# EasyVision-Ton/VMG

Measured on AMD Instinct MI355X. Metric: LR-frames/s (train: forward+loss+backward+AdamW), VMG-REDS-few_levels 4x SR, higher is better.
Workload: dtype bf16; 1 GPU; VMG-REDS-few_levels train step, per-GPU batch 4x7x3x64x64 -> 4x SR (BASELINE configs[1]); global_batch=4, frames_per_clip=7, parallelism=dp1, launch=eager, recompute_chains=False, fp8_chains=False

## Files before the change

### include/vmg_hip.h

```cpp
#ifndef VMG_HIP_H
#define VMG_HIP_H

#include <stdint.h>

#ifdef __cplusplus
extern "C" {
#endif

#define VMG_F32 0
#define VMG_BF16 1

#define VMG_ACT_NONE 0
#define VMG_ACT_RELU 1
#define VMG_ACT_LRELU 2
#define VMG_ACT_GELU 3

#define VMG_CONV_GENERAL 0
#define VMG_CONV_KSPLIT 2
#define VMG_CONV_WS 3
#define VMG_CONV_LINEAR_WRES 4
#define VMG_CONV_WSTAT 6

const char* vmg_last_error(void);
int vmg_version(void);

typedef struct vmg_ctx vmg_ctx;
vmg_ctx* vmg_create(int device);
int vmg_destroy(vmg_ctx* ctx);
int vmg_ctx_device(const vmg_ctx* ctx);
int vmg_max_lds_bytes(void);

int64_t vmg_conv_pack_bytes(int dtype, int ks, int on, int nsrc, const int* src_ch, int cout_tiles);
int vmg_conv_pack(int dtype, const float* w, int O, int I, int ks, int o0, int on, int nsrc, const int* src_off,
                  const int* src_ch, int transpose_flip, int cout_tiles, void* packed, void* stream);

int64_t vmg_convws_pack_bytes(int on, int nsrc, const int* src_ch, int cout_tiles);
int vmg_convws_pack(const float* w, int O, int I, int o0, int on, int nsrc, const int* src_off, const int* src_ch, int transpose_flip,
                    int cout_tiles, void* packed, void* stream);

typedef struct vmg_conv_desc {
  int dtype, ks, cout_tiles;
  int N, H, W, Cout;
  int nsrc;
  const void* src[4];
  int64_t src_ps[4];
  int src_ch[4];
  const void* packed;
  const float* bias;
  void* out;
  int64_t out_ps;
  void* out_pre;
  const void* res;
  int64_t res_ps;
  const void* aux;
// ... 269 lines not shown
```

### vmg_amd/csrc/conv_igemm.hip

```cpp
#include <stdlib.h>

#include <type_traits>

#include "common.h"

namespace {

constexpr int MAX_ISRC = 32;
constexpr int CBMAX = 160;

__host__ __device__ constexpr int kstg(int ks) { return ks > 1 ? ks : 2; }
__host__ __device__ constexpr int stage_bytes(int ks, int ntb, int cb) { return kstg(ks) * 4 * ntb * 16 * cb; }
__host__ __device__ constexpr int stage_stride(int ks, int ntb, int cb) { return (stage_bytes(ks, ntb, cb) + 4095) / 4096 * 4096; }
__host__ __device__ inline int stages_of(int ks, int ch) {
  const int nb = (ch / 8 + 3) / 4;
  return ks > 1 ? ks * nb : (nb + 1) / 2;
}

struct ConvK {
  const char* src[MAX_ISRC];
  long long src_ps[MAX_ISRC];
  short src_ch[MAX_ISRC];
  short src_nst[MAX_ISRC];
  int src_pixb[MAX_ISRC];
// ... 1341 lines not shown
      } else if (a.act == VMG_ACT_RELU) {
#pragma unroll
        for (int r = 0; r < 8; ++r) v[r] = fmaxf(v[r], 0.f);
      } else if (a.act == VMG_ACT_LRELU) {
#pragma unroll
        for (int r = 0; r < 8; ++r) v[r] = v[r] > 0.f ? v[r] : v[r] * a.slope;
      }
      if (a.alpha != 1.0f) {
#pragma unroll
        for (int r = 0; r < 8; ++r) v[r] *= a.alpha;
      }
      if (auxb) {
        bf16x8 u = pre[it];
        if (a.res) u = *reinterpret_cast<const bf16x8*>(auxb + opix * (int)a.aux_ps + c8 * 8);
#pragma unroll
        for (int r = 0; r < 8; ++r) {
          const float uf = (float)u[r];
          v[r] *= a.actgrad == 3 ? gelu_erf_grad(uf) : (uf > 0.f ? 1.f : (a.actgrad == 2 ? a.slope : 0.f));
        }
      }
      if (a.res) {
#pragma unroll
        for (int r = 0; r < 8; ++r) v[r] += (float)pre[it][r];
      }
      bf16x8 tq;
#pragma unroll
      for (int r = 0; r < 8; ++r) tq[r] = (bf16)v[r];
      __builtin_nontemporal_store(tq, reinterpret_cast<bf16x8*>(out + opix * (int)a.out_ps + c8 * 8));
    }
  }
  ws_stamp(a, wave, 31);
}

struct PackK {
  const float* w;
  char* out;
  int O, I, ks, o0, on, nsrc, transpose_flip, cob, ncb, nstages, ss_elems;
  int groups;
  int fast3;
  long long units;
  short src_off[MAX_ISRC], src_ch[MAX_ISRC], src_st0[MAX_ISRC], src_nst[MAX_ISRC];
};

__device__ __forceinline__ float pack_weight_value(const PackK& p, int oc, int kc, int tap, int KK) {
  if (p.groups <= 1) {
    if (!p.transpose_flip) return p.w[((long long)oc * p.I + kc) * KK + tap];
    return p.w[((long long)kc * p.I + oc) * KK + (KK - 1 - tap)];
  }
  const int og = p.O / p.groups;
  if (!p.transpose_flip) {
    const int kl = kc - (oc / og) * p.I;
    return (kl >= 0 && kl < p.I) ? p.w[((long long)oc * p.I + kl) * KK + tap] : 0.f;
  }
  const int g = oc / p.I;
  return (kc / og == g) ? p.w[((long long)kc * p.I + (oc - g * p.I)) * KK + (KK - 1 - tap)] : 0.f;
}

template <typename T>
__device__ __forceinline__ void pack_std_vec8(const PackK& p, long long i8) {
  const unsigned i = (unsigned)i8 * 8u;
  const int KK = p.ks * p.ks, KSTG = kstg(p.ks);
  const int body = KSTG * 4 * p.cob * 8;
  const unsigned r = i / (unsigned)p.ss_elems;
  const int within = (int)(i - r * (unsigned)p.ss_elems);
  const int cb = (int)(r / (unsigned)p.nstages);
  const int stage = (int)(r - (unsigned)cb * (unsigned)p.nstages);
// ... 365 lines not shown
  int nwg = vmg_cu_count(dev) & ~7;
  if (nwg < 8) nwg = 8;
  while (nwg > 8 && (long long)(nwg >> 3) > cdiv64(ntiles, 8)) nwg -= 8;
  hipLaunchKernelGGL(fn, dim3((unsigned)nwg, ncb), dim3(512), lds, st, k, (int)ntiles);
  VMG_LAUNCH_CHECK();
  return 0;
}

template <int NCT, int NB>
int launch_wstat(const ConvK& k, int ncb, hipStream_t st) {
  const bool full = k.res || k.aux || k.out_pre || k.act == VMG_ACT_GELU;
  return full ? launch_wstat2<NCT, NB, true>(k, ncb, st) : launch_wstat2<NCT, NB, false>(k, ncb, st);
}

template <int NCT>
int launch_ws(const ConvK& k, int ncb, hipStream_t st) {
  using G = WsGeo<NCT>;
  ConvK kk = k;
  kk.ring = NCT <= 3 ? 3 : ((k.halo_bytes + 4 * G::STG + G::COB * 4 <= 160 * 1024) ? 4 : 3);
  const int lds = k.halo_bytes + kk.ring * G::STG + G::COB * 4;
  VMG_CHECK(lds <= 160 * 1024, "conv (weight-streaming): LDS request %d B exceeds 160 KiB", lds);
  auto fn = conv_ws_kernel<NCT>;
  static bool attr_set[VMG_MAX_DEVICES] = {};
  const int dev = vmg_current_device();
  if (!attr_set[dev]) {
    (void)hipFuncSetAttribute(reinterpret_cast<const void*>(fn), hipFuncAttributeMaxDynamicSharedMemorySize, 160 * 1024);
    attr_set[dev] = true;
  }
  const long long nblk = (long long)k.N * k.tiles_y * k.tiles_x;
  VMG_CHECK(nblk > 0 && nblk < (1ll << 31), "conv: bad grid %lld", nblk);
  const bool prof = (k.nsrc == 1 && k.src_ch[0] == k.Cout && (k.Cout == 144 || k.Cout == 112)) && vmg_prof_before(VMG_PROF_CONV3X3, k.M, st);
  hipLaunchKernelGGL(fn, dim3((unsigned)nblk, ncb), dim3(G::THREADS), lds, st, kk);
  if (prof) vmg_prof_after(st);
  VMG_LAUNCH_CHECK();
  return 0;
}

}

#ifdef VMG_DIAG
static unsigned long long* g_conv_stamps = nullptr;
#endif
extern "C" int vmg_conv_debug_stamps(void* buf) {
#ifdef VMG_DIAG
  g_conv_stamps = (unsigned long long*)buf;
  return 0;
#else
  (void)buf;
  vmg_set_error("conv_debug_stamps: this library was built without -DVMG_DIAG (VMG_DIAG=1 python -m vmg_amd.build)");
  return -1;
#endif
}

extern "C" int64_t vmg_conv_pack_bytes(int dtype, int ks, int on, int nsrc, const int* src_ch, int cout_tiles) {
  short xoff[MAX_ISRC], xch[MAX_ISRC];
  const int n = expand_sources(nsrc, nullptr, src_ch, xoff, xch, nullptr);
  if (n < 0 || cout_tiles <= 0 || (ks != 1 && ks != 3 && ks != 7)) return -1;
  int64_t nst = 0;
  for (int s = 0; s < n; ++s) nst += stages_of(ks, xch[s]);
  const int cob = cout_tiles * 16;
  const int ncb = (on + cob - 1) / cob;
  return (int64_t)ncb * nst * stage_stride(ks, cout_tiles, dtype == VMG_BF16 ? 16 : 32);
}

static int fill_pack_std(PackK& p, long long& total, int dtype, const float* w, int O, int I, int ks, int o0, int on, int nsrc, const int* src_off,
                         const int* src_ch, int transpose_flip, int cout_tiles, void* packed) {
// ... 134 lines not shown
  int rc;
  if (kind == 1) {
    VMG_CHECK(ks == 3 && dtype == VMG_BF16, "pack_entry: the weight-streaming layout is bf16 3x3");
    rc = fill_pack_ws(e.p, e.total, w, O, I, o0, on, nsrc, src_off, src_ch, transpose_flip, cout_tiles, packed);
  } else {
    rc = fill_pack_std(e.p, e.total, dtype, w, O, I, ks, o0, on, nsrc, src_off, src_ch, transpose_flip, cout_tiles, packed);
  }
  if (rc) return rc;
  e.kind = kind; e.dtype = dtype; e.blk0 = blk0;
  long long nb = e.p.fast3 ? (e.p.units + 255) / 256 : (e.total + 256LL * 16 - 1) / (256LL * 16);
  e.nblk = (int)(nb < 1 ? 1 : (nb > 64 ? 64 : nb));
  memcpy(entry, &e, sizeof(e));
  return e.nblk;
}

extern "C" int vmg_pack_run(const void* plan_dev, int n, int total_blocks, void* stream) {
  VMG_CHECK(plan_dev && n > 0 && total_blocks > 0, "pack_run: bad arguments");
  static_assert(sizeof(PackEntry) % 4 == 0, "the block-owner table sits behind the entries");
  hipLaunchKernelGGL(pack_batch_kernel, dim3(total_blocks), dim3(256), 0, (hipStream_t)stream, (const PackEntry*)plan_dev, n);
  VMG_LAUNCH_CHECK();
  return 0;
}

extern "C" int vmg_conv_fwd(const vmg_conv_desc* d, void* stream) {
  VMG_CHECK(d != nullptr, "conv_fwd: null descriptor");
  VMG_CHECK(d->ks == 1 || d->ks == 3 || d->ks == 7, "conv_fwd: ks must be 1, 3 or 7");
  VMG_CHECK(d->dtype == VMG_F32 || d->dtype == VMG_BF16, "conv_fwd: bad dtype");
  VMG_CHECK(d->nsrc >= 1 && d->nsrc <= 4, "conv_fwd: nsrc must be 1..4");
  VMG_CHECK(d->N > 0 && d->H > 0 && d->W > 0 && d->Cout > 0, "conv_fwd: bad shape");
  VMG_CHECK(d->packed && d->out, "conv_fwd: null packed weights / output");
  VMG_CHECK(!d->pixel_shuffle || (d->Cout % 4 == 0), "conv_fwd: pixel_shuffle needs Cout %% 4 == 0");
  VMG_CHECK(!(d->actgrad != 0 && d->aux == nullptr), "conv_fwd: actgrad without aux");
  VMG_CHECK(d->deep == VMG_CONV_GENERAL || d->deep == VMG_CONV_KSPLIT || d->deep == VMG_CONV_WS || d->deep == VMG_CONV_LINEAR_WRES ||
                d->deep == VMG_CONV_WSTAT,
            "conv_fwd: unknown kernel route deep = %d", d->deep);
  const int es = d->dtype == VMG_BF16 ? 2 : 4, cbytes = es * 8;
  ConvK k;
  memset(&k, 0, sizeof(k));
  short xoff[MAX_ISRC];
  int parent[MAX_ISRC];
  const int n = expand_sources(d->nsrc, nullptr, d->src_ch, xoff, k.src_ch, parent);
  VMG_CHECK(n > 0, "conv_fwd: source channel counts must be multiples of 8");
  int mt = d->mt;
  if (d->dtype == VMG_F32) mt = 1;
  const long long M = (long long)d->N * d->H * d->W;
  const int ntb = d->cout_tiles;
  VMG_CHECK(ntb > 0, "conv_fwd: cout_tiles must be positive");
  const int ncb = cdiv(d->Cout, ntb * 16);
  if (d->ks == 7) mt = 1;
  if (mt == 0) mt = 1;
  VMG_CHECK(mt == 1 || mt == 2, "conv_fwd: mt must be 1 or 2");
  const int TH = 4 * mt, TWH = 16 + d->ks - 1, THH = TH + d->ks - 1;
  int kt = 0, halo = 0;
  for (int s = 0; s < n; ++s) {
    const int par = parent[s];
    VMG_CHECK(d->src[par] != nullptr, "conv_fwd: null source %d", par);
    VMG_CHECK(d->src_ps[par] >= d->src_ch[par] && (d->src_ps[par] * es) % 16 == 0, "conv_fwd: source pixel stride must be >= channels and 16-byte aligned");
    VMG_CHECK(((uintptr_t)d->src[par]) % 16 == 0, "conv_fwd: source pointer must be 16-byte aligned");
    k.src[s] = (const char*)d->src[par] + (long long)xoff[s] * es;
    k.src_ps[s] = d->src_ps[par];
    k.src_nst[s] = (short)stages_of(d->ks, k.src_ch[s]);
    k.src_pixb[s] = choose_pixb(k.src_ch[s], es, cbytes);
    kt += k.src_nst[s];
    const int hb = THH * TWH * k.src_pixb[s];
    if (hb > halo) halo = hb;
  }
  k.nsrc = n;
  k.wpack = (const char*)d->packed; k.bias = d->bias;
  k.out = (char*)d->out; k.out_ps = d->out_ps; k.out_pre = (char*)d->out_pre;
  k.res = (const char*)d->res; k.res_ps = d->res_ps; k.aux = (const char*)d->aux; k.aux_ps = d->aux_ps;
  k.N = d->N; k.H = d->H; k.W = d->W; k.Cout = d->Cout; k.M = M;
  k.tiles_x = cdiv(d->W, 16); k.tiles_y = cdiv(d->H, TH);
  k.act = d->act; k.slope = d->slope; k.alpha = d->alpha; k.actgrad = d->aux ? d->actgrad : 0; k.ps = d->pixel_shuffle;
#ifdef VMG_DIAG
  {
    const char* e = getenv("VMG_CONV_DBG");
    k.dbg = e ? atoi(e) : 0;
    k.stamps = g_conv_stamps;
  }
#endif
  {
    auto al = [](const void* p) { return ((uintptr_t)p & 15) == 0; };
    k.vec8 = d->dtype == VMG_BF16 && !d->pixel_shuffle && (d->Cout % 16) == 0 && (d->out_ps % 8) == 0 && al(d->out) &&
             (!d->out_pre || al(d->out_pre)) && (!d->res || ((d->res_ps % 8) == 0 && al(d->res))) &&
             (!d->aux || ((d->aux_ps % 8) == 0 && al(d->aux)));
  }
  k.nstages = kt; k.halo_bytes = (halo + 1023) & ~1023;
  VMG_CHECK(d->out_ps >= (d->pixel_shuffle ? d->Cout / 4 : d->Cout), "conv_fwd: out pixel stride too small");
  hipStream_t st = (hipStream_t)stream;
  if (d->deep == VMG_CONV_WS) {
    VMG_CHECK(d->dtype == VMG_BF16 && d->ks == 3 && k.vec8 && (ntb == 3 || ntb == 7 || ntb == 8 || ntb == 9), "conv_fwd: the weight-streaming kernel is bf16 3x3 with 16-byte aligned rows, cout_tiles 3, 7, 8 or 9");
    for (int s = 0; s < n; ++s) VMG_CHECK(k.src_ch[s] % 16 == 0, "conv_fwd: the weight-streaming kernel takes channel blocks that are multiples of 16 (got %d)", k.src_ch[s]);
    int kt3 = 0, halo3 = 0;
    for (int s = 0; s < n; ++s) {
      k.src_pixb[s] = k.src_ch[s] * 2;
      k.src_nst[s] = (short)(ws_ksteps(k.src_ch[s] >> 3) / 3);
      kt3 += k.src_nst[s];
      const int hb = 10 * 18 * k.src_pixb[s];
      if (hb > halo3) halo3 = hb;
    }
    k.nstages = kt3;
    k.halo_bytes = (halo3 + 1023) & ~1023;
    k.tiles_y = cdiv(d->H, 8);
    return ntb == 9 ? launch_ws<9>(k, ncb, st) : (ntb == 7 ? launch_ws<7>(k, ncb, st) : (ntb == 8 ? launch_ws<8>(k, ncb, st) : launch_ws<3>(k, ncb, st)));
  }
  if (d->deep == VMG_CONV_WSTAT && d->dtype == VMG_BF16 && d->ks == 3 && mt == 1 && k.vec8 && n == 1 && (ntb == 1 || ntb == 3 || ntb == 4) && k.src_ch[0] <= 64 && k.src_ch[0] % 8 == 0 &&
      k.src_ps[0] % 8 == 0 && d->W <= 255 * 16 && (long long)d->W * k.src_ps[0] * 2 * 10 < (1ll << 31)) {
    ConvK kk = k;
    kk.tiles_y = cdiv(d->H, 8);
    const int nb = (k.src_ch[0] / 8 + 3) / 4;
    switch (ntb * 2 + (nb - 1)) {
      case 2: return launch_wstat<1, 1>(kk, ncb, st);
      case 3: return launch_wstat<1, 2>(kk, ncb, st);
      case 6: return launch_wstat<3, 1>(kk, ncb, st);
      case 7: return launch_wstat<3, 2>(kk, ncb, st);
      case 8: return launch_wstat<4, 1>(kk, ncb, st);
      case 9: return launch_wstat<4, 2>(kk, ncb, st);
    }
  }
  if (d->deep == VMG_CONV_LINEAR_WRES && d->dtype == VMG_BF16 && d->ks == 1 && k.vec8 && (ntb == 3 || ntb == 5)) {
    if (n == 1 && k.src_ch[0] <= 160 && k.src_pixb[0] == k.src_ch[0] * 2) return ntb == 3 ? launch_linear_wres<3>(k, ncb, st) : launch_linear_wres<5>(k, ncb, st);
    if (n == 2 && ntb == 3 && d->nsrc == 1 && k.src_ch[0] == k.src_ch[1] && k.src_ch[0] <= 160 && k.src[1] == k.src[0] + k.src_ch[0] * 2 &&
        k.src_nst[0] == k.src_nst[1])
      return launch_linear_wres<3, 2>(k, ncb, st);
  }
  if (d->ks == 7) return d->dtype == VMG_BF16 ? dispatch_ks7<bf16>(k, ntb, ncb, st) : dispatch_ks7<float>(k, ntb, ncb, st);
  if (d->deep == VMG_CONV_KSPLIT) {
    VMG_CHECK(d->dtype == VMG_BF16 && mt == 1, "conv_fwd: the k-split variant is bf16, mt = 1");
    return d->ks == 3 ? dispatch_ksplit<bf16, 3>(k, ntb, ncb, k.halo_bytes, st) : dispatch_ksplit<bf16, 1>(k, ntb, ncb, k.halo_bytes, st);
  }
  if (d->dtype == VMG_BF16) {
    if (d->ks == 3) return mt == 2 ? dispatch_ntb<bf16, 3, 2>(k, ntb, ncb, st) : dispatch_ntb<bf16, 3, 1>(k, ntb, ncb, st);
    return mt == 2 ? dispatch_ntb<bf16, 1, 2>(k, ntb, ncb, st) : dispatch_ntb<bf16, 1, 1>(k, ntb, ncb, st);
  }
  if (d->ks == 3) return dispatch_ntb<float, 3, 1>(k, ntb, ncb, st);
  return dispatch_ntb<float, 1, 1>(k, ntb, ncb, st);
// ... 47 lines not shown
```

### vmg_amd/functional.py

```python
from __future__ import annotations

import contextlib
from typing import List, Optional, Sequence

import torch

from . import hip
from . import kernels as K
from .hip import HipError
from .wgrad import DEFERRED, _wgrad_entries, _wgrad_now, flush_deferred_wgrads, recorded, set_wgrad_mode

class _Fn(torch.autograd.Function):

    @classmethod
    def apply(cls, *args):
        return super(torch.autograd.Function, cls).apply(*args)


def _pad_to(n: int, m: int = 8) -> int:
    return (n + m - 1) // m * m


def choose_tiling(M: int, cout: int, ks: int, dtype: torch.dtype, src_ch: Optional[Sequence[int]] = None, pixel_shuffle: bool = False):
    if USE_WS and src_ch is not None and not pixel_shuffle:
        t = K.ws_eligible(cout, ks, dtype, src_ch)
        if t and M <= 16384 and cout in (112, 144):
            return (4 if cout == 112 else 3), 1, hip.CONV_KSPLIT
        if t:
            return t, 1, hip.CONV_WS
    if dtype == torch.bfloat16 and ks == 3 and cout in (144, 288):
        return 3, 1, hip.CONV_KSPLIT
    if dtype == torch.bfloat16 and ks == 1 and src_ch is not None and len(src_ch) == 1 and M >= 65536 and not pixel_shuffle:
        if cout == 144 and src_ch[0] == 144:
            return 5, 1, hip.CONV_LINEAR_WRES
        if cout == 288 and src_ch[0] == 144:
            return 5, 1, hip.CONV_LINEAR_WRES
        if cout == 144 and src_ch[0] == 288:
            return 3, 1, hip.CONV_LINEAR_WRES
    if dtype == torch.bfloat16 and ks == 3 and not pixel_shuffle and M >= (1 << 18) and src_ch is not None and len(src_ch) == 1 and \
            src_ch[0] <= 64 and src_ch[0] % 8 == 0 and cout in (16, 48, 64):
        return cout // 16, 1, hip.CONV_WSTAT
    if dtype == torch.bfloat16 and ks == 3 and not pixel_shuffle and M >= (1 << 20) and src_ch is not None and len(src_ch) == 1 and \
            (cout <= 16 or src_ch[0] <= 16):
        return None, 2, hip.CONV_GENERAL
    return None, 1, hip.CONV_GENERAL


USE_WS = True
GROUPED_DENSE = True

class _PlanState:

    def __init__(self):
        self.plan, self.stamp, self.wkey, self.ents, self.packs = K.PackPlan(), -1, None, [], []


def _from_param(ent) -> bool:
    pw, weight = ent[1], ent[2]
    return pw.call is not None and pw.call[0] == weight.data_ptr()


class _PackCache:

    def __init__(self):
        self.ents = {}
        self.q8 = {}
        self.volatile = set()
        self.epoch = 0
        self.stamp = 0
        self.stable = _PlanState()
        self.vol = _PlanState()
        self.decay = None

    def get(self, key, weight: torch.Tensor, build, planned: bool = True):
        ents = self.ents if planned else self.q8
        ver = (weight._version, self.epoch)
        hit = ents.get(key)
        buf = None
        if hit is not None:
            if hit[2] is weight:
                if hit[0] == ver:
# ... 37 lines not shown

    def repack_all(self):
        self._run_plan(self.stable, None, lambda key, ent: key not in self.volatile and _from_param(ent))

    def decay_weights_and_repack(self, weights: Sequence[torch.Tensor], gammas: Sequence[torch.Tensor], n: int = 1):
        wkey = tuple(map(id, weights))
        if weights[0].is_cuda:
            dkey = (wkey, tuple(map(id, gammas)))
            if self.decay is None or self.decay[0] != dkey:
                self.decay = (dkey, K.DecayList(weights, gammas))
            self.decay[1].run(n)
        else:
            with torch.no_grad():
                for _ in range(int(n)):
                    torch._foreach_mul_(list(weights), list(gammas))
        ids = set(wkey)
        self._run_plan(self.vol, wkey, lambda key, ent: key in self.volatile and id(ent[2]) in ids and _from_param(ent), reset_sig=True)


PACKS = _PackCache()
clear_pack_cache = PACKS.clear
bump_weight_epoch = PACKS.bump_epoch
repack_all = PACKS.repack_all
decay_weights_and_repack = PACKS.decay_weights_and_repack


def _pack_image(ws: bool, w: torch.Tensor, dtype: torch.dtype, **kw) -> K.PackedConv:
    return K.pack_conv_weight_ws(w, **kw) if ws else K.pack_conv_weight(w, dtype, **kw)


def packed(weight: torch.Tensor, dtype: torch.dtype, kind: str, src_ch: Optional[Sequence[int]] = None,
           i0: int = 0, on: Optional[int] = None, tiles: Optional[int] = None, deep: int = hip.CONV_GENERAL, orange: Optional[Sequence[int]] = None,
           groups: int = 1) -> K.PackedConv:
    ws = deep == hip.CONV_WS
    if groups > 1:
        return PACKS.get((id(weight), kind, dtype, "dense", groups, tiles, ws), weight, _build_grouped_dense)
    key = (id(weight), kind, dtype, tuple(src_ch) if src_ch else None, i0, on, tiles, ws, tuple(orange) if orange else None)
    return PACKS.get(key, weight, _build_pack)


def _build_pack(key, weight: torch.Tensor, buf: Optional[torch.Tensor]) -> K.PackedConv:
    _, kind, dtype, src_ch, i0, on, tiles, ws, orange = key
    w = weight.detach()
    if w.dim() == 2:
        w = w[:, :, None, None]
    O, I = w.shape[0], w.shape[1]
    if kind == "fwd":
        if src_ch is None:
            src_ch = [I]
        if sum(src_ch) != I:
            raise HipError(f"source channels {list(src_ch)} do not sum to weight input channels {I}")
        if any(c % 8 for c in src_ch):
            parts, off = [], 0
            for c in src_ch:
                parts.append((off, c))
                off += c
            wp = w.new_zeros(O, sum(_pad_to(c) for _, c in parts), *w.shape[2:])
            po = 0
            for o_, c in parts:
                wp[:, po:po + c] = w[:, o_:o_ + c]
                po += _pad_to(c)
            w = wp
            src_ch = [_pad_to(c) for c in src_ch]
        o0, no = (orange[0], orange[1]) if orange else (0, None)
        return _pack_image(ws, w.contiguous(), dtype, src_ch=list(src_ch), cout_tiles=tiles, o0=o0, on=no, out=buf)
    if kind == "dgrad":
        on = I - i0 if on is None else on
# ... 35 lines not shown

def _act_grad(dy: torch.Tensor, y: Optional[torch.Tensor], pre: Optional[torch.Tensor], act: int, slope: float, alpha: float):
    if act == hip.ACT_NONE:
        return dy if alpha == 1.0 else dy * alpha
    return K.act_backward(dy, pre if act == hip.ACT_GELU else y, act, slope, alpha)


class _ActTok:
    __slots__ = ("act", "slope", "alpha", "pre", "masked")

    def __init__(self, act, slope, alpha):
        self.act, self.slope, self.alpha, self.pre, self.masked = act, slope, alpha, None, False


_ACTGRAD_CODE = {hip.ACT_RELU: 1, hip.ACT_LRELU: 2, hip.ACT_GELU: 3}


class _Conv2d(_Fn):

    @staticmethod
    def forward(ctx, weight, bias, res, cfg, *srcs):
        ks, act, slope, alpha, pixel_shuffle, N, H, W, tok, src_tok = cfg
        cfg = cfg[:8]
        ctx.tok, ctx.src_tok = tok, src_tok
        dt = srcs[0].dtype
        src_ch = [s.shape[-1] for s in srcs]
        srcs_p = [_pad_channels(s) for s in srcs]
        tiles, mt, deep = choose_tiling(N * H * W, weight.shape[0], ks, dt, src_ch, pixel_shuffle)
        ps_after = False
        if pixel_shuffle and USE_WS and res is None:
            t_ws = K.ws_eligible(weight.shape[0], ks, dt, [s.shape[-1] for s in srcs_p])
            if t_ws:
                ps_after, tiles, mt, deep = True, t_ws, 1, hip.CONV_WS
        pw = packed(weight, dt, "fwd", src_ch, tiles=tiles, deep=deep)
        need_pre = act == hip.ACT_GELU and any(ctx.needs_input_grad)
        out, pre = K.conv_forward(srcs_p, pw, bias, N, H, W, act=act, slope=slope, alpha=alpha, res=res,
                                  pixel_shuffle=pixel_shuffle and not ps_after, want_pre=need_pre, mt=mt, deep=deep)
        if ps_after:
            out = K.pixel_shuffle(out, N, H, W)
        if tok is not None:
            tok.pre = pre
        ctx.cfg = cfg
        ctx.src_ch = src_ch
        ctx.src_shapes = [tuple(t.shape) for t in srcs]
        ctx.res_shape = tuple(res.shape) if res is not None else None
        ctx.has_res = res is not None
        ctx.has_bias = bias is not None
        ctx.defer = DEFERRED.defers(weight, bias, ctx.needs_input_grad[0])
        if ctx.defer:
            ctx.gen = DEFERRED.note_use(weight, bias)
            ctx.bias_ref = bias
        if act in (hip.ACT_RELU, hip.ACT_LRELU) and res is not None:
            raise HipError("activation + residual in one epilogue is not differentiable from the output alone")
        ctx.save_for_backward(weight, out if act in (hip.ACT_RELU, hip.ACT_LRELU) else None, pre, *srcs_p)
        return out

    @staticmethod
    def backward(ctx, dy):
        ks, act, slope, alpha, pixel_shuffle, N, H, W = ctx.cfg
        weight, y, pre = ctx.saved_tensors[:3]
        srcs_p = ctx.saved_tensors[3:]
        dy = dy.contiguous()
        d_res = dy.reshape(ctx.res_shape) if ctx.has_res else None
        if ctx.tok is not None and ctx.tok.masked:
            ctx.tok.masked = False
            dpre = dy
# ... 1163 lines not shown
```

### vmg_amd/hip.py

```python
from __future__ import annotations

import ctypes
import os
from ctypes import POINTER, c_char_p, c_float, c_int, c_int64, c_void_p

import torch

HERE = os.path.dirname(os.path.abspath(__file__))
LIB_PATH = os.environ.get("VMG_HIP_LIB") or os.path.join(HERE, "libvmg_hip.so")

F32, BF16 = 0, 1
ACT_NONE, ACT_RELU, ACT_LRELU, ACT_GELU = 0, 1, 2, 3
CONV_GENERAL, CONV_KSPLIT, CONV_WS, CONV_LINEAR_WRES, CONV_WSTAT = 0, 2, 3, 4, 6
WGRAD_V1, WGRAD_3, WGRAD_3B, WGRAD_L2, WGRAD_7 = 1, 2, 3, 4, 5


def wgrad_kernel_id(kind: int, a: int = 0, b: int = 0, c: int = 0) -> int:
    return kind << 24 | a << 16 | b << 8 | c


class HipError(RuntimeError):
    pass


class ConvDesc(ctypes.Structure):
    _fields_ = [
        ("dtype", c_int), ("ks", c_int), ("cout_tiles", c_int),
        ("N", c_int), ("H", c_int), ("W", c_int), ("Cout", c_int),
        ("nsrc", c_int),
        ("src", c_void_p * 4), ("src_ps", c_int64 * 4), ("src_ch", c_int * 4),
        ("packed", c_void_p), ("bias", c_void_p),
        ("out", c_void_p), ("out_ps", c_int64), ("out_pre", c_void_p),
        ("res", c_void_p), ("res_ps", c_int64),
        ("aux", c_void_p), ("aux_ps", c_int64),
        ("act", c_int), ("slope", c_float), ("alpha", c_float),
        ("actgrad", c_int), ("pixel_shuffle", c_int), ("mt", c_int), ("deep", c_int),
    ]


class ChainDesc(ctypes.Structure):
    _fields_ = [
        ("dtype", c_int), ("N", c_int), ("H", c_int), ("W", c_int), ("C", c_int), ("nblk", c_int), ("nsrc", c_int),
        ("src", c_void_p * 4), ("src_ps", c_int64 * 4), ("src_ch", c_int * 4),
        ("packed0", c_void_p), ("bias0", c_void_p), ("slope0", c_float), ("cout_tiles0", c_int), ("deep0", c_int),
        ("packed1", POINTER(c_void_p)), ("bias1", POINTER(c_void_p)), ("packed2", POINTER(c_void_p)), ("bias2", POINTER(c_void_p)),
        ("r_scaling", c_float), ("cout_tiles", c_int), ("deep", c_int),
# ... 229 lines not shown
```

### vmg_amd/kernels.py

```python
from __future__ import annotations

import ctypes
import os
import struct
from typing import Optional, Sequence, Tuple

import torch

from . import hip
from .hip import ConvDesc, HipError


def _intarr(v: Sequence[int]):
    return (ctypes.c_int * len(v))(*[int(x) for x in v])


def cout_tiles_for(cout: int, dtype: torch.dtype = torch.bfloat16, ks: int = 3) -> int:
    t = (cout + 15) // 16
    if t <= 1:
        return 1
    if ks == 7:
        return 2 if t == 2 else 4
    if t <= 4:
        return 4
# ... 46 lines not shown
        raise HipError(f"vmg_conv_pack_bytes rejected channels {list(src_ch)} (must be multiples of 8)")
    if out is None:
        out = torch.empty(nbytes, dtype=torch.uint8, device=w.device)
    elif out.numel() * out.element_size() < nbytes:
        raise HipError("pack buffer too small")
    hip.check(l.vmg_conv_pack(code, w.data_ptr(), O, I, ks, o0, on, len(src_ch), _intarr(src_off), _intarr(src_ch),
                              flag, tiles, out.data_ptr(), hip.stream_ptr()), "vmg_conv_pack")
    return PackedConv(out, dtype, ks, on, src_ch, tiles, call=(w.data_ptr(), O, I, o0, on, list(src_off), list(src_ch), flag))


WS_128_BLOCKS = os.environ.get("VMG_WS_128", "1") != "0"


def ws_eligible(cout: int, ks: int, dtype: torch.dtype, src_ch: Sequence[int]) -> int:
    if dtype != torch.bfloat16 or ks != 3:
        return 0
    for c in src_ch:
        parts = 1
        while c // parts > 160 or c % (8 * parts):
            parts += 1
            if parts > c // 8:
                return 0
        if (c // parts) % 16:
            return 0
    if cout % 144 == 0:
        return 9
    if cout % 112 == 0:
        return 7
    if cout % 128 == 0 and WS_128_BLOCKS:
        return 8
    return 0


def pack_conv_weight_ws(w: torch.Tensor, src_ch: Optional[Sequence[int]] = None, src_off: Optional[Sequence[int]] = None, o0: int = 0,
                        on: Optional[int] = None, transpose_flip: bool = False, cout_tiles: int = 9, out: Optional[torch.Tensor] = None,
                        groups: int = 1) -> PackedConv:
    hip.require_cuda(w)
    if w.dtype != torch.float32 or not w.is_contiguous() or w.dim() != 4 or w.shape[2] != 3 or w.shape[3] != 3:
        raise HipError("pack_conv_weight_ws expects a contiguous fp32 (O, I, 3, 3) weight")
    O, I = w.shape[0], w.shape[1]
    kdim, odim = (O, I * groups) if transpose_flip else (I * groups, O)
    if src_ch is None:
        src_ch, src_off = [kdim], [0]
    if src_off is None:
        src_off, acc = [], 0
        for c in src_ch:
            src_off.append(acc)
            acc += c
    if on is None:
        on = odim - o0
    flag = (1 if transpose_flip else 0) | ((groups << 8) if groups > 1 else 0)
    l = hip.lib()
    nbytes = l.vmg_convws_pack_bytes(on, len(src_ch), _intarr(src_ch), cout_tiles)
    if nbytes <= 0:
        raise HipError(f"vmg_convws_pack_bytes rejected channels {list(src_ch)} / cout_tiles {cout_tiles}")
    if out is None:
        out = torch.empty(nbytes, dtype=torch.uint8, device=w.device)
    elif out.numel() * out.element_size() < nbytes:
        raise HipError("pack buffer too small")
    hip.check(l.vmg_convws_pack(w.data_ptr(), O, I, o0, on, len(src_ch), _intarr(src_off), _intarr(src_ch), flag,
                                cout_tiles, out.data_ptr(), hip.stream_ptr()), "vmg_convws_pack")
    return PackedConv(out, torch.bfloat16, 3, on, src_ch, cout_tiles, layout="ws",
                      call=(w.data_ptr(), O, I, o0, on, list(src_off), list(src_ch), flag))


_CONV_FMT = struct.Struct("=8i4Q4q4iQQQqQQqQqiffiiii4x")
# ... 2 lines not shown
_CONV_PACK = _CONV_FMT.pack_into


def _pix_stride(t: torch.Tensor) -> int:
    st = t.stride()
    if st[-1] != 1:
        raise HipError("channels must be the fastest dimension")
    if t.is_contiguous():
        return t.shape[-1]
    sh = t.shape
    ps = st[-2]
    expect = ps
    for d in range(len(sh) - 2, -1, -1):
        if sh[d] != 1 and st[d] != expect:
            raise HipError(f"tensor of shape {tuple(sh)} / strides {st} is not a dense pixel array")
        expect *= sh[d]
    return ps


def conv_forward(srcs: Sequence[torch.Tensor], pw: PackedConv, bias: Optional[torch.Tensor], N: int, H: int, W: int,
                 act: int = hip.ACT_NONE, slope: float = 0.0, alpha: float = 1.0, res: Optional[torch.Tensor] = None,
                 aux: Optional[torch.Tensor] = None, actgrad: int = 0, pixel_shuffle: bool = False,
                 out: Optional[torch.Tensor] = None, out_pre: Optional[torch.Tensor] = None, want_pre: bool = False,
                 mt: int = 0, deep: int = hip.CONV_GENERAL) -> Tuple[torch.Tensor, Optional[torch.Tensor]]:
    if len(srcs) != len(pw.src_ch):
        raise HipError(f"conv expects {len(pw.src_ch)} sources, got {len(srcs)}")
    x0 = srcs[0]
    hip.require_cuda(*srcs, bias, res, aux, out)
    dt = x0.dtype
    if dt != pw.dtype:
        raise HipError(f"activation dtype {dt} != packed weight dtype {pw.dtype}")
    M = N * H * W
    nsrc = len(srcs)
    if (pw.layout == "ws") != (deep == hip.CONV_WS):
        deep = hip.CONV_WS if pw.layout == "ws" else hip.CONV_GENERAL
    sp, sps, sch = [0, 0, 0, 0], [0, 0, 0, 0], [0, 0, 0, 0]
    for i, s in enumerate(srcs):
        if s.dtype != dt or s.shape[-1] != pw.src_ch[i] or s.numel() // s.shape[-1] != M:
            raise HipError(f"source {i}: shape {tuple(s.shape)} / dtype {s.dtype} does not match conv (M={M}, C={pw.src_ch[i]}, {dt})")
        sp[i], sps[i], sch[i] = s.data_ptr(), _pix_stride(s), pw.src_ch[i]
    bias_p = 0
    if bias is not None:
        if bias.dtype != torch.float32 or bias.numel() != pw.cout or not bias.is_contiguous():
            raise HipError("bias must be contiguous fp32 of length Cout")
        bias_p = bias.data_ptr()
    if pixel_shuffle:
        oshape = (N, 2 * H, 2 * W, pw.cout // 4)
    else:
        oshape = (N, H, W, pw.cout)
    if out is None:
        out = torch.empty(oshape, dtype=dt, device=x0.device)
    elif out.dtype != dt or out.numel() // out.shape[-1] != (4 * M if pixel_shuffle else M) or out.shape[-1] != oshape[-1]:
        raise HipError(f"bad output tensor {tuple(out.shape)} for conv output {oshape}")
    out_ps = _pix_stride(out)
    if want_pre and out_pre is None:
        if pixel_shuffle:
            raise HipError("out_pre is not available with pixel_shuffle")
        out_pre = torch.empty(oshape, dtype=dt, device=x0.device)
    pre_p = 0
    if out_pre is not None:
        if _pix_stride(out_pre) != out_ps or out_pre.shape[-1] != pw.cout or out_pre.dtype != dt:
            raise HipError("out_pre must have the layout of out")
        pre_p = out_pre.data_ptr()
    extra = [0, 0, 0, 0]
    for k, (name, t) in enumerate((("res", res), ("aux", aux))):
        if t is None:
            continue
# ... 1262 lines not shown
```

Before: 582.5 LR-frames/s.

## Add tile-pair weight-streaming 3x3 conv kernel covering 16 rows per block

Adds a second weight-streaming bf16 3x3 conv kernel in which each 512-thread block covers a 16x16 output tile. Each wave computes two pixel rows, so every streamed weight stage is reused over twice as many pixels. The weight ring is double-buffered and the epilogue is staged through LDS. A Python heuristic picks this route only when the halved block count saves enough scheduling rounds across the 256 CUs, using a fixed 1.87 per-round cost factor. The trade-off is a larger halo, more LDS and fewer blocks, which can hurt occupancy and tail balance.

Measured after the change: 586.5 LR-frames/s, median of 6. About the same (+0.7%).

```diff
diff --git a/include/vmg_hip.h b/include/vmg_hip.h
--- a/include/vmg_hip.h
+++ b/include/vmg_hip.h
@@ -20,6 +20,7 @@
 #define VMG_CONV_WS 3
 #define VMG_CONV_LINEAR_WRES 4
 #define VMG_CONV_WSTAT 6
+#define VMG_CONV_WS2 8
 
 const char* vmg_last_error(void);
 int vmg_version(void);
diff --git a/vmg_amd/csrc/conv_igemm.hip b/vmg_amd/csrc/conv_igemm.hip
--- a/vmg_amd/csrc/conv_igemm.hip
+++ b/vmg_amd/csrc/conv_igemm.hip
@@ -1397,6 +1397,289 @@
   ws_stamp(a, wave, 31);
 }
 
+template <int NCT>
+struct Ws2Geo {
+  static constexpr int COB = NCT * 16, KSB = COB * 64, STG = 3 * KSB;
+  static constexpr int TH = 16, TWH = 18, THH = 18, THREADS = 512, NP = 3 * NCT;
+  static constexpr int C8 = 2 * NCT, TOTAL = 256 * C8, NIT = TOTAL / THREADS, PSTR = WsItems<NCT>::PSTR;
+  static_assert(TOTAL % THREADS == 0, "whole items per thread");
+  static_assert(TOTAL <= 5000, "WsItems::decode is exact below 5461");
+  __host__ __device__ static constexpr int lds_bytes(int halo_bytes) {
+    return halo_bytes + 2 * STG + COB * 4 > 256 * PSTR ? halo_bytes + 2 * STG + COB * 4 : 256 * PSTR;
+  }
+};
+
+template <int NCT>
+__global__ __launch_bounds__(512, 2) void conv_ws2_kernel(const ConvK a) {
+  using G = Ws2Geo<NCT>;
+  using T = bf16;
+  constexpr int COB = G::COB, KSB = G::KSB, STG = G::STG;
+  extern __shared__ __attribute__((aligned(16))) char smem[];
+  char* halo = smem;
+  char* ring = smem + a.halo_bytes;
+  float* lbias = reinterpret_cast<float*>(ring + 2 * STG);
+  const int tid = threadIdx.x, lane = tid & 63;
+  const int wave = __builtin_amdgcn_readfirstlane(tid >> 6);
+  const int cb = blockIdx.y;
+  const int bid = xcd_remap(blockIdx.x, gridDim.x, 0);
+  const int tx = bid % a.tiles_x;
+  const int rr = bid / a.tiles_x;
+  const int ty = rr % a.tiles_y, n = rr / a.tiles_y;
+  const int nstages = a.nstages;
+  const int px = lane & 15, g = lane >> 4;
+
+  auto issue_halo = [&](int s) {
+    const int ch = a.src_ch[s];
+    const char* sp = a.src[s];
+    const int ps32 = (int)(a.src_ps[s] * 2);
+    const int vpp = ch >> 3, row_vecs = G::TWH * vpp, total = G::THH * row_vecs;
+    const float inv_row = 1.0f / (float)row_vecs, inv_vpp = 1.0f / (float)vpp;
+    const int y0 = ty * G::TH - 1, x0 = tx * 16 - 1;
+    const char* origin = sp + (((long long)n * a.H + y0) * a.W + x0) * (long long)ps32;
+    const int rowstep = a.W * ps32;
+    const int nq = a.halo_bytes >> 10;
+    for (int q = wave; q < nq; q += 8) {
+      const int L = q * 64 + lane;
+      const int r = (int)(((float)L + 0.5f) * inv_row);
+      const int rem = L - r * row_vecs;
+      const int p = (int)(((float)rem + 0.5f) * inv_vpp);
+      const int v = rem - p * vpp;
+      const bool ok = (L < total) & ((unsigned)(y0 + r) < (unsigned)a.H) & ((unsigned)(x0 + p) < (unsigned)a.W);
+      const char* gp = ok ? origin + (long long)(r * rowstep + p * ps32 + v * 16) : reinterpret_cast<const char*>(&g_conv_zero16);
+      glds16_asm(gp, halo + q * 1024);
+    }
+  };
+
+  const char* wsrc = a.wpack + ((long long)cb * nstages) * STG + lane * 16;
+  const int prot = bid % G::NP;
+  auto issue_stage = [&](int gst, int sl) {
+    const char* gsrc = wsrc + (long long)gst * STG;
+    char* dst = ring + sl * STG;
+#pragma unroll
+    for (int i = 0; i < (G::NP + 7) / 8; ++i) {
+      const int q = wave + 8 * i;
+      if (q < G::NP) {
+        int ii = q + prot;
+        ii = ii >= G::NP ? ii - G::NP : ii;
+        glds16_asm(gsrc + ii * 1024, dst + ii * 1024);
+      }
+    }
+  };
+
+  int cs = 0, csl = 0, cst0 = 0, cnst = a.src_nst[0], crot = bid % cnst;
+  int slot = 0;
+  auto issue_succ = [&]() {
+    if (csl + 1 < cnst) {
+      issue_stage(cst0 + (crot + 1 == cnst ? 0 : crot + 1), slot ^ 1);
+    } else if (cs + 1 < a.nsrc) {
+      issue_stage(cst0 + cnst + bid % a.src_nst[cs + 1], slot ^ 1);
+    }
+  };
+
+  issue_halo(0);
+  issue_stage(crot, 0);
+  if (tid < COB) lbias[tid] = (a.bias && cb * COB + tid < a.Cout) ? a.bias[cb * COB + tid] : 0.f;
+
+  f32x4 acc[NCT][2];
+  Frag<T> wf[3][NCT], xf[3][2];
+  int CH = a.src_ch[0] >> 3, nfull3 = 3 * (CH >> 2), pixb = a.src_pixb[0], rowb = G::TWH * pixb;
+  const char* xb = halo + ((2 * wave) * G::TWH + px) * pixb;
+  int xo[3];
+  auto stage_offsets = [&]() {
+    if (crot < nfull3) {
+      const int cbk = (crot * 171) >> 9, ky = crot - 3 * cbk;
+      const int base = ky * rowb + cbk * 64 + g * 16;
+      xo[0] = base; xo[1] = base + pixb; xo[2] = base + 2 * pixb;
+    } else {
+      const int nfull = CH >> 2, jr0 = 3 * (crot - nfull3);
+#pragma unroll
+      for (int jj = 0; jj < 3; ++jj) {
+        int tap = 2 * (jr0 + jj) + (g >> 1);
+        tap = tap > 8 ? 8 : tap;
+        const int tyy = (tap * 11) >> 5;
+        xo[jj] = tyy * rowb + (tap - 3 * tyy) * pixb + (4 * nfull + (g & 1)) * 16;
+      }
+    }
+  };
+  auto advance = [&]() {
+    ++csl;
+    crot = crot + 1 == cnst ? 0 : crot + 1;
+    slot ^= 1;
+  };
+  auto next_source = [&]() {
+    ++cs;
+    cst0 += cnst;
+    csl = 0; cnst = a.src_nst[cs]; crot = bid % cnst;
+    CH = a.src_ch[cs] >> 3; nfull3 = 3 * (CH >> 2); pixb = a.src_pixb[cs]; rowb = G::TWH * pixb;
+    xb = halo + ((2 * wave) * G::TWH + px) * pixb;
+    slot ^= 1;
+  };
+  auto rd = [&](int set, int jj) {
+    xf[set][0].load(xb + xo[jj]);
+    xf[set][1].load(xb + rowb + xo[jj]);
+    const char* wp = ring + slot * STG + jj * KSB + g * (COB * 16) + px * 16;
+#pragma unroll
+    for (int ct = 0; ct < NCT; ++ct) wf[set][ct].load(wp + ct * 256);
+  };
+  auto mm = [&](int set) {
+#pragma unroll
+    for (int ct = 0; ct < NCT; ++ct) {
+      acc[ct][0] = mma(wf[set][ct], xf[set][0], acc[ct][0]);
+      acc[ct][1] = mma(wf[set][ct], xf[set][1], acc[ct][1]);
+    }
+  };
+  auto phase_fence = [&]() {
+#pragma unroll
+    for (int i = 0; i < NCT + 2; ++i) {
+      __builtin_amdgcn_sched_group_barrier(0x008, 1, 0);
+      __builtin_amdgcn_sched_group_barrier(0x100, 1, 0);
+    }
+    __builtin_amdgcn_sched_group_barrier(0x008, 2 * NCT - (NCT + 2), 0);
+    __builtin_amdgcn_sched_barrier(0);
+  };
+  auto stage_wait = [&]() {
+    __builtin_amdgcn_s_waitcnt(0xC07F);
+    asm volatile("s_waitcnt vmcnt(0)" ::: "memory");
+  };
+
+  asm volatile("s_waitcnt vmcnt(0)\n\ts_waitcnt lgkmcnt(0)" ::: "memory");
+  __builtin_amdgcn_s_barrier();
+  asm volatile("" ::: "memory");
+  issue_succ();
+#pragma unroll
+  for (int ct = 0; ct < NCT; ++ct) {
+    const f32x4 bv = *reinterpret_cast<const f32x4*>(lbias + ct * 16 + g * 4);
+    acc[ct][0] = bv;
+    acc[ct][1] = bv;
+  }
+  stage_offsets();
+  rd(0, 0);
+  __builtin_amdgcn_sched_barrier(0);
+  for (int s = 0; s < a.nsrc; ++s) {
+    for (int sl = 0; sl + 1 < cnst; ++sl) {
+      rd(1, 1);
+      mm(0);
+      phase_fence();
+      rd(2, 2);
+      mm(1);
+      phase_fence();
+      stage_wait();
+      __builtin_amdgcn_s_barrier();
+      asm volatile("" ::: "memory");
+      advance();
+      issue_succ();
+      stage_offsets();
+      rd(0, 0);
+      mm(2);
+      phase_fence();
+    }
+    rd(1, 1);
+    mm(0);
+    phase_fence();
+    rd(2, 2);
+    mm(1);
+    phase_fence();
+    stage_wait();
+    __builtin_amdgcn_s_barrier();
+    asm volatile("" ::: "memory");
+    if (s + 1 < a.nsrc) issue_halo(s + 1);
+    mm(2);
+    __builtin_amdgcn_sched_barrier(0);
+    if (s + 1 < a.nsrc) {
+      asm volatile("s_waitcnt vmcnt(0)" ::: "memory");
+      __builtin_amdgcn_s_barrier();
+      asm volatile("" ::: "memory");
+      next_source();
+      issue_succ();
+      stage_offsets();
+      rd(0, 0);
+      __builtin_amdgcn_sched_barrier(0);
+    }
+  }
+
+  const long long tile_pix = ((long long)n * a.H + ty * G::TH) * a.W + tx * 16;
+  const bf16* esrc = reinterpret_cast<const bf16*>(a.res ? a.res : a.aux);
+  bf16x8 pre[G::NIT];
+  if (esrc) {
+    const long long eps = a.res ? a.res_ps : a.aux_ps;
+    const bf16* ebase = esrc + tile_pix * eps + cb * COB;
+#pragma unroll
+    for (int it = 0; it < G::NIT; ++it) {
+      int pxl, c8;
+      WsItems<NCT>::decode(it * G::THREADS + tid, pxl, c8);
+      const int row = pxl >> 4, col = pxl & 15;
+      const bool valid = (ty * G::TH + row < a.H) & (tx * 16 + col < a.W) & (cb * COB + c8 * 8 < a.Cout);
+      const int off = valid ? (row * a.W + col) * (int)eps + c8 * 8 : 0;
+      pre[it] = *reinterpret_cast<const bf16x8*>(ebase + off);
+    }
+  }
+  {
+    char* prow = smem + ((2 * wave) * 16 + px) * G::PSTR + g * 16;
+#pragma unroll
+    for (int ct = 0; ct < NCT; ++ct) {
+      *reinterpret_cast<f32x4*>(prow + ct * 64) = acc[ct][0];
+      *reinterpret_cast<f32x4*>(prow + 16 * G::PSTR + ct * 64) = acc[ct][1];
+    }
+    __builtin_amdgcn_s_waitcnt(0xC07F);
+  }
+  __builtin_amdgcn_s_barrier();
+  asm volatile("" ::: "memory");
+  {
+    bf16* out = reinterpret_cast<bf16*>(a.out) + tile_pix * a.out_ps + cb * COB;
+    bf16* out_pre = a.out_pre ? reinterpret_cast<bf16*>(a.out_pre) + tile_pix * a.out_ps + cb * COB : nullptr;
+    const bf16* auxb = a.aux ? reinterpret_cast<const bf16*>(a.aux) + tile_pix * a.aux_ps + cb * COB : nullptr;
+#pragma unroll
+    for (int it = 0; it < G::NIT; ++it) {
+      int pxl, c8;
+      WsItems<NCT>::decode(it * G::THREADS + tid, pxl, c8);
+      const int row = pxl >> 4, col = pxl & 15;
+      const bool valid = (ty * G::TH + row < a.H) & (tx * 16 + col < a.W) & (cb * COB + c8 * 8 < a.Cout);
+      if (!valid) continue;
+      const char* pp = smem + pxl * G::PSTR + c8 * 32;
+      const f32x4 lo = *reinterpret_cast<const f32x4*>(pp), hi = *reinterpret_cast<const f32x4*>(pp + 16);
+      float v[8] = {lo[0], lo[1], lo[2], lo[3], hi[0], hi[1], hi[2], hi[3]};
+      const int opix = row * a.W + col;
+      if (out_pre) {
+        bf16x8 tq;
+#pragma unroll
+        for (int r = 0; r < 8; ++r) tq[r] = (bf16)v[r];
+        *reinterpret_cast<bf16x8*>(out_pre + opix * (int)a.out_ps + c8 * 8) = tq;
+      }
+      if (a.act == VMG_ACT_GELU) {
+#pragma unroll
+        for (int r = 0; r < 8; ++r) v[r] = gelu_erf(v[r]);
+      } else if (a.act == VMG_ACT_RELU) {
+#pragma unroll
+        for (int r = 0; r < 8; ++r) v[r] = fmaxf(v[r], 0.f);
+      } else if (a.act == VMG_ACT_LRELU) {
+#pragma unroll
+        for (int r = 0; r < 8; ++r) v[r] = v[r] > 0.f ? v[r] : v[r] * a.slope;
+      }
+      if (a.alpha != 1.0f) {
+#pragma unroll
+        for (int r = 0; r < 8; ++r) v[r] *= a.alpha;
+      }
+      if (auxb) {
+        bf16x8 u = pre[it];
+        if (a.res) u = *reinterpret_cast<const bf16x8*>(auxb + opix * (int)a.aux_ps + c8 * 8);
+#pragma unroll
+        for (int r = 0; r < 8; ++r) {
+          const float uf = (float)u[r];
+          v[r] *= a.actgrad == 3 ? gelu_erf_grad(uf) : (uf > 0.f ? 1.f : (a.actgrad == 2 ? a.slope : 0.f));
+        }
+      }
+      if (a.res) {
+#pragma unroll
+        for (int r = 0; r < 8; ++r) v[r] += (float)pre[it][r];
+      }
+      bf16x8 tq;
+#pragma unroll
+      for (int r = 0; r < 8; ++r) tq[r] = (bf16)v[r];
+      __builtin_nontemporal_store(tq, reinterpret_cast<bf16x8*>(out + opix * (int)a.out_ps + c8 * 8));
+    }
+  }
+}
+
 struct PackK {
   const float* w;
   char* out;
@@ -1828,6 +2111,25 @@
   const bool prof = (k.nsrc == 1 && k.src_ch[0] == k.Cout && (k.Cout == 144 || k.Cout == 112)) && vmg_prof_before(VMG_PROF_CONV3X3, k.M, st);
   hipLaunchKernelGGL(fn, dim3((unsigned)nblk, ncb), dim3(G::THREADS), lds, st, kk);
   if (prof) vmg_prof_after(st);
+  VMG_LAUNCH_CHECK();
+  return 0;
+}
+
+template <int NCT>
+int launch_ws2(const ConvK& k, int ncb, hipStream_t st) {
+  using G = Ws2Geo<NCT>;
+  const int lds = G::lds_bytes(k.halo_bytes);
+  VMG_CHECK(lds <= 160 * 1024, "conv (weight-streaming, tile pairs): LDS request %d B exceeds 160 KiB", lds);
+  auto fn = conv_ws2_kernel<NCT>;
+  static bool attr_set[VMG_MAX_DEVICES] = {};
+  const int dev = vmg_current_device();
+  if (!attr_set[dev]) {
+    (void)hipFuncSetAttribute(reinterpret_cast<const void*>(fn), hipFuncAttributeMaxDynamicSharedMemorySize, 160 * 1024);
+    attr_set[dev] = true;
+  }
+  const long long nblk = (long long)k.N * k.tiles_y * k.tiles_x;
+  VMG_CHECK(nblk > 0 && nblk < (1ll << 31), "conv: bad grid %lld", nblk);
+  hipLaunchKernelGGL(fn, dim3((unsigned)nblk, ncb), dim3(G::THREADS), lds, st, k);
   VMG_LAUNCH_CHECK();
   return 0;
 }
@@ -2028,7 +2330,7 @@
   VMG_CHECK(!d->pixel_shuffle || (d->Cout % 4 == 0), "conv_fwd: pixel_shuffle needs Cout %% 4 == 0");
   VMG_CHECK(!(d->actgrad != 0 && d->aux == nullptr), "conv_fwd: actgrad without aux");
   VMG_CHECK(d->deep == VMG_CONV_GENERAL || d->deep == VMG_CONV_KSPLIT || d->deep == VMG_CONV_WS || d->deep == VMG_CONV_LINEAR_WRES ||
-                d->deep == VMG_CONV_WSTAT,
+                d->deep == VMG_CONV_WSTAT || d->deep == VMG_CONV_WS2,
             "conv_fwd: unknown kernel route deep = %d", d->deep);
   const int es = d->dtype == VMG_BF16 ? 2 : 4, cbytes = es * 8;
   ConvK k;
@@ -2084,20 +2386,22 @@
   k.nstages = kt; k.halo_bytes = (halo + 1023) & ~1023;
   VMG_CHECK(d->out_ps >= (d->pixel_shuffle ? d->Cout / 4 : d->Cout), "conv_fwd: out pixel stride too small");
   hipStream_t st = (hipStream_t)stream;
-  if (d->deep == VMG_CONV_WS) {
-    VMG_CHECK(d->dtype == VMG_BF16 && d->ks == 3 && k.vec8 && (ntb == 3 || ntb == 7 || ntb == 8 || ntb == 9), "conv_fwd: the weight-streaming kernel is bf16 3x3 with 16-byte aligned rows, cout_tiles 3, 7, 8 or 9");
+  if (d->deep == VMG_CONV_WS || d->deep == VMG_CONV_WS2) {
+    const bool pair = d->deep == VMG_CONV_WS2;
+    VMG_CHECK(d->dtype == VMG_BF16 && d->ks == 3 && k.vec8 && ((ntb == 3 && !pair) || ntb == 7 || ntb == 8 || ntb == 9), "conv_fwd: the weight-streaming kernel is bf16 3x3 with 16-byte aligned rows, cout_tiles 3 (one-tile form only), 7, 8 or 9");
     for (int s = 0; s < n; ++s) VMG_CHECK(k.src_ch[s] % 16 == 0, "conv_fwd: the weight-streaming kernel takes channel blocks that are multiples of 16 (got %d)", k.src_ch[s]);
     int kt3 = 0, halo3 = 0;
     for (int s = 0; s < n; ++s) {
       k.src_pixb[s] = k.src_ch[s] * 2;
       k.src_nst[s] = (short)(ws_ksteps(k.src_ch[s] >> 3) / 3);
       kt3 += k.src_nst[s];
-      const int hb = 10 * 18 * k.src_pixb[s];
+      const int hb = (pair ? 18 : 10) * 18 * k.src_pixb[s];
       if (hb > halo3) halo3 = hb;
     }
     k.nstages = kt3;
     k.halo_bytes = (halo3 + 1023) & ~1023;
-    k.tiles_y = cdiv(d->H, 8);
+    k.tiles_y = cdiv(d->H, pair ? 16 : 8);
+    if (pair) return ntb == 9 ? launch_ws2<9>(k, ncb, st) : (ntb == 7 ? launch_ws2<7>(k, ncb, st) : launch_ws2<8>(k, ncb, st));
     return ntb == 9 ? launch_ws<9>(k, ncb, st) : (ntb == 7 ? launch_ws<7>(k, ncb, st) : (ntb == 8 ? launch_ws<8>(k, ncb, st) : launch_ws<3>(k, ncb, st)));
   }
   if (d->deep == VMG_CONV_WSTAT && d->dtype == VMG_BF16 && d->ks == 3 && mt == 1 && k.vec8 && n == 1 && (ntb == 1 || ntb == 3 || ntb == 4) && k.src_ch[0] <= 64 && k.src_ch[0] % 8 == 0 &&
diff --git a/vmg_amd/functional.py b/vmg_amd/functional.py
--- a/vmg_amd/functional.py
+++ b/vmg_amd/functional.py
@@ -26,6 +26,8 @@
         t = K.ws_eligible(cout, ks, dtype, src_ch)
         if t and M <= 16384 and cout in (112, 144):
             return (4 if cout == 112 else 3), 1, hip.CONV_KSPLIT
+        if t and USE_WS2 and K.ws2_eligible(M, cout, ks, dtype, src_ch):
+            return t, 1, hip.CONV_WS2
         if t:
             return t, 1, hip.CONV_WS
     if dtype == torch.bfloat16 and ks == 3 and cout in (144, 288):
@@ -47,6 +49,7 @@
 
 
 USE_WS = True
+USE_WS2 = True
 GROUPED_DENSE = True
 
 class _PlanState:
@@ -150,7 +153,7 @@
 def packed(weight: torch.Tensor, dtype: torch.dtype, kind: str, src_ch: Optional[Sequence[int]] = None,
            i0: int = 0, on: Optional[int] = None, tiles: Optional[int] = None, deep: int = hip.CONV_GENERAL, orange: Optional[Sequence[int]] = None,
            groups: int = 1) -> K.PackedConv:
-    ws = deep == hip.CONV_WS
+    ws = deep in (hip.CONV_WS, hip.CONV_WS2)
     if groups > 1:
         return PACKS.get((id(weight), kind, dtype, "dense", groups, tiles, ws), weight, _build_grouped_dense)
     key = (id(weight), kind, dtype, tuple(src_ch) if src_ch else None, i0, on, tiles, ws, tuple(orange) if orange else None)
@@ -252,6 +255,8 @@
             t_ws = K.ws_eligible(weight.shape[0], ks, dt, [s.shape[-1] for s in srcs_p])
             if t_ws:
                 ps_after, tiles, mt, deep = True, t_ws, 1, hip.CONV_WS
+                if USE_WS2 and K.ws2_eligible(N * H * W, weight.shape[0], ks, dt, [s.shape[-1] for s in srcs_p]):
+                    deep = hip.CONV_WS2
         pw = packed(weight, dt, "fwd", src_ch, tiles=tiles, deep=deep)
         need_pre = act == hip.ACT_GELU and any(ctx.needs_input_grad)
         out, pre = K.conv_forward(srcs_p, pw, bias, N, H, W, act=act, slope=slope, alpha=alpha, res=res,
diff --git a/vmg_amd/hip.py b/vmg_amd/hip.py
--- a/vmg_amd/hip.py
+++ b/vmg_amd/hip.py
@@ -11,7 +11,7 @@
 
 F32, BF16 = 0, 1
 ACT_NONE, ACT_RELU, ACT_LRELU, ACT_GELU = 0, 1, 2, 3
-CONV_GENERAL, CONV_KSPLIT, CONV_WS, CONV_LINEAR_WRES, CONV_WSTAT = 0, 2, 3, 4, 6
+CONV_GENERAL, CONV_KSPLIT, CONV_WS, CONV_LINEAR_WRES, CONV_WSTAT, CONV_WS2 = 0, 2, 3, 4, 6, 8
 WGRAD_V1, WGRAD_3, WGRAD_3B, WGRAD_L2, WGRAD_7 = 1, 2, 3, 4, 5
 
 
diff --git a/vmg_amd/kernels.py b/vmg_amd/kernels.py
--- a/vmg_amd/kernels.py
+++ b/vmg_amd/kernels.py
@@ -102,6 +102,22 @@
     return 0
 
 
+NUM_CUS = 256
+WS2_ROUND_COST = 1.87
+WS2_MAX_PIXELS = 1 << 22
+
+
+def ws2_eligible(M: int, cout: int, ks: int, dtype: torch.dtype, src_ch: Sequence[int]) -> int:
+    t = ws_eligible(cout, ks, dtype, src_ch)
+    tiles = (M + 127) // 128
+    if not t or tiles <= NUM_CUS or M > WS2_MAX_PIXELS:
+        return 0
+    ncb = (cout + 16 * t - 1) // (16 * t)
+    rounds_one = (tiles * ncb + NUM_CUS - 1) // NUM_CUS
+    rounds_pair = ((M + 255) // 256 * ncb + NUM_CUS - 1) // NUM_CUS
+    return t if rounds_pair * WS2_ROUND_COST < rounds_one else 0
+
+
 def pack_conv_weight_ws(w: torch.Tensor, src_ch: Optional[Sequence[int]] = None, src_off: Optional[Sequence[int]] = None, o0: int = 0,
                         on: Optional[int] = None, transpose_flip: bool = False, cout_tiles: int = 9, out: Optional[torch.Tensor] = None,
                         groups: int = 1) -> PackedConv:
@@ -170,7 +186,7 @@
         raise HipError(f"activation dtype {dt} != packed weight dtype {pw.dtype}")
     M = N * H * W
     nsrc = len(srcs)
-    if (pw.layout == "ws") != (deep == hip.CONV_WS):
+    if (pw.layout == "ws") != (deep in (hip.CONV_WS, hip.CONV_WS2)):
         deep = hip.CONV_WS if pw.layout == "ws" else hip.CONV_GENERAL
     sp, sps, sch = [0, 0, 0, 0], [0, 0, 0, 0], [0, 0, 0, 0]
     for i, s in enumerate(srcs):
```
